# vLAR-group/unMORE

Measured on AMD Instinct MI355X. Metric: images/sec (train fwd+bwd) ObjectnessNet ViT-B/16 384x384, higher is better.
Workload: dtype bf16

## Files before the change

### unmore_amd/csrc/gemm_nt256p.hip

```cpp
#include "umr_common.h"
#include "gemm_epilogue.h"
#include <stdio.h>
#include <stdlib.h>
#include <type_traits>

namespace {

constexpr int BM2 = 256, BN2 = 256, BK2 = 64;
constexpr int ROWB2 = 128;
constexpr int TILE2 = 256 * ROWB2;
constexpr int BUF2 = 2 * TILE2;
constexpr int STG_OFF = 2 * BUF2;
constexpr int STG_BYTES = 32 * 256 * 4;
constexpr int LDS2P = STG_OFF + STG_BYTES;

typedef bf16_t T2;

__device__ __forceinline__ unsigned mul_dgelu_bf16x2(unsigned g, unsigned x) {
    const float lo = __builtin_bit_cast(float, g << 16) * dgelu_sel<bf16_t>(__builtin_bit_cast(float, x << 16));
    const float hi = __builtin_bit_cast(float, g & 0xFFFF0000u) * dgelu_sel<bf16_t>(__builtin_bit_cast(float, x & 0xFFFF0000u));
    typedef __attribute__((ext_vector_type(2))) __bf16 bf16x2;
    bf16x2 r;
    r[0] = (bf16_t)lo; r[1] = (bf16_t)hi;
    return __builtin_bit_cast(unsigned, r);
// ... 313 lines not shown
        QUADRANT_HID(0, fb0, (void)0, (void)0)
        END_SYNC_N(2);
    };
    auto tile_body4_ahead = [&](const char* sbuf) {
#pragma unroll
        for (int ks = 0; ks < 2; ++ks) {
#pragma unroll
            for (int i = 0; i < 2; ++i) fb0[ks][i] = B_FRAG(ks, i);
#pragma unroll
            for (int i = 0; i < 4; ++i) fa[ks][i] = A_FRAG(ks, i);
        }
        READ_WAIT();
        QUADRANT(0, 0, fb0, 1)
        END_SYNC_N(6);
#pragma unroll
        for (int ks = 0; ks < 2; ++ks)
#pragma unroll
            for (int i = 0; i < 2; ++i) fb1[ks][i] = B_FRAG(ks, 2 + i);
        READ_WAIT();
        QUADRANT(0, 2, fb1, 2)
        END_SYNC_N(6);
#pragma unroll
        for (int ks = 0; ks < 2; ++ks)
#pragma unroll
            for (int i = 0; i < 4; ++i) fa[ks][i] = A_FRAG(ks, 4 + i);
        READ_WAIT();
        QUADRANT(4, 2, fb1, 3)
        END_SYNC_N(6);
        stage_prep();
        QUADRANT(4, 0, fb0, 0)
        END_SYNC_N(6);
    };

    if (PRIO_MODE == 1 && w >= 4) __builtin_amdgcn_s_setprio(1);
    stage_setup(0);
    stage_prep();
    STAGE_DMA(0, 0); STAGE_DMA(0, 1); STAGE_DMA(1, 0); STAGE_DMA(1, 1);
    STAGE_DMA(2, 0); STAGE_DMA(2, 1); STAGE_DMA(3, 0); STAGE_DMA(3, 1);
    if (ahead) {
        if (PH2) {
            asm volatile("s_waitcnt vmcnt(2)" ::: "memory");
        } else {
            stage_prep();
            STAGE_DMA(0, 0); STAGE_DMA(0, 1);
            asm volatile("s_waitcnt vmcnt(6)" ::: "memory");
        }
    } else {
        stage_prep();
        STAGE_DMA(0, 0); STAGE_DMA(0, 1); STAGE_DMA(1, 0); STAGE_DMA(1, 1);
        if (PH2) { STAGE_DMA(2, 0); STAGE_DMA(2, 1); }
        asm volatile("s_waitcnt vmcnt(8)" ::: "memory");
    }
    __builtin_amdgcn_s_barrier();

    const int er = lane >> 3, ec = lane & 7;
    const unsigned co_lane = ((unsigned)((w >> 2) * 128 + er) * (unsigned)p.ldc + (unsigned)((w & 3) * 64 + ec * 8)) * 2u;
    const unsigned ax_lane = ((unsigned)((w >> 2) * 128 + er) * (unsigned)p.ldaux + (unsigned)((w & 3) * 64 + ec * 8)) * 2u;
    constexpr int WST_BYTES = 2048;
    constexpr int RW_OFF = 8 * WST_BYTES;
    float* stg = (float*)(smem + STG_OFF);
    auto stage_rows = [&](auto mtag) {
        constexpr int MT = decltype(mtag)::value;
        const int lr = wr * 16 + frow;
#pragma unroll
        for (int ntl = 0; ntl < 4; ++ntl) {
            const int ch = (wc * 16 + ntl * 4 + fq) ^ frow;
            *(f32x4*)(stg + lr * 256 + ch * 4) = acc[MT][ntl];
        }
    };
    int c_par = 0;
    constexpr bool BIAS_INIT = (EPI == 3 || EPI == 4 || EPI == 5 || EPI == 6);
    f32x4 bqn[4];
    auto fetch_bias = [&](int it_) {
        const int v_ = it_ * G + pw;
        const int tn_ = v_ - (v_ / tiles_n) * tiles_n;
#pragma unroll
        for (int ntl = 0; ntl < 4; ++ntl) {
            const int n = tn_ * BN2 + wc * 64 + ntl * 16 + fq * 4;
            bqn[ntl] = f32x4{0.f, 0.f, 0.f, 0.f};
            if ((p.flags & UMR_EPI_BIAS) && it_ < n_my && n < p.N) bqn[ntl] = *(const f32x4*)(p.bias + n);
        }
    };
    if (BIAS_INIT) fetch_bias(0);
#pragma unroll 1
    for (int it = 0; it < n_my; ++it) {
#pragma unroll
        for (int i = 0; i < 8; ++i)
#pragma unroll
            for (int j = 0; j < 4; ++j) acc[i][j] = BIAS_INIT ? bqn[j] : f32x4{0.f, 0.f, 0.f, 0.f};
        if (RED && w < 2) {
            const int v_ = it * G + pw;
            const int n0_ = (v_ - (v_ / tiles_n) * tiles_n) * BN2;
            const __amdgpu_buffer_rsrc_t rsW = __builtin_amdgcn_make_buffer_rsrc(
                (void*)(p.red_w + (int64_t)w * p.N + n0_), 0, (w < p.red_c) ? clamp31((int64_t)(p.N - n0_) * 4) : 0, 0x00020000);
            const int rw_off = (EPI == 3) ? RW_OFF + (it & 1) * 2048 : 0;
            __builtin_amdgcn_raw_ptr_buffer_load_lds(rsW, UMR_LDS_PTR(smem + STG_OFF + rw_off + w * 1024), 16, (unsigned)(lane * 16), 0, 0, 0);
        }
        if (ahead) {
#pragma unroll 1
            for (int t = 0; t < nt; ++t) {
                if (PH2) tile_body2_ahead(smem + c_par * BUF2); else tile_body4_ahead(smem + c_par * BUF2);
                c_par ^= 1;
            }
        } else {
#pragma unroll 1
            for (int t = 0; t < nt; ++t) {
                tile_body(smem + c_par * BUF2);
                c_par ^= 1;
            }
        }
        const int v = it * G + pw;
        const int tm = v / tiles_n, tn = v - tm * tiles_n;
        const int m0 = tm * bm, n0 = tn * BN2;
        const int m_end = (p.M - m0 < bm) ? p.M : m0 + bm;
        if (EPI == 3) {
            fetch_bias(it + 1);
            typedef __attribute__((ext_vector_type(2))) short s16x2;
            typedef __attribute__((ext_vector_type(2))) unsigned u32x2;
            const short relu_lo = (p.act == UMR_ACT_RELU) ? (short)0 : (short)-32768;
            const s16x2 relu16 = {relu_lo, relu_lo};
            auto pack4 = [&](const f32x4& v) -> u32x2 {
                unsigned lo, hi;
                asm("v_cvt_pk_bf16_f32 %0, %1, %2" : "=v"(lo) : "v"(v[0]), "v"(v[1]));
                asm("v_cvt_pk_bf16_f32 %0, %1, %2" : "=v"(hi) : "v"(v[2]), "v"(v[3]));
                s16x2 a = __builtin_bit_cast(s16x2, lo), b = __builtin_bit_cast(s16x2, hi);
                if (AUXM == 0) {
                    a = __builtin_elementwise_max(a, relu16);
                    b = __builtin_elementwise_max(b, relu16);
                }
                return u32x2{__builtin_bit_cast(unsigned, a), __builtin_bit_cast(unsigned, b)};
            };
            bf16x8 rwh[2], rwl[2];
            float* ro_lane = nullptr;
            if (RED) {
#pragma unroll
                for (int pr = 0; pr < 2; ++pr) {
                    f32x4 a = {0.f, 0.f, 0.f, 0.f}, b = {0.f, 0.f, 0.f, 0.f};
                    if (frow < 2) {
                        const char* rwp = smem + STG_OFF + RW_OFF + (it & 1) * 2048 + frow * 1024;
                        a = *(const f32x4*)(rwp + (wc * 64 + (2 * pr) * 16 + fq * 4) * 4);
                        b = *(const f32x4*)(rwp + (wc * 64 + (2 * pr + 1) * 16 + fq * 4) * 4);
                    }
#pragma unroll
                    for (int e = 0; e < 8; ++e) {
                        const float x = e < 4 ? a[e] : b[e - 4];
                        const bf16_t hi = (bf16_t)x;
                        rwh[pr][e] = hi;
                        rwl[pr][e] = (bf16_t)(x - (float)hi);
                    }
                }
                if (fq == 0 && n0 + wc * 64 < p.N)
                    ro_lane = p.red_out + ((int64_t)(tn * 4 + wc) * p.M + (m0 + wr * 128 + frow)) * p.red_c;
            }
            auto row_reduce2 = [&](const bf16x8& a01, const bf16x8& a23, const bf16x8& b01, const bf16x8& b23, int mt_) {
                const f32x4 z = {0.f, 0.f, 0.f, 0.f};
                f32x4 ra = __builtin_amdgcn_mfma_f32_16x16x32_bf16(rwh[0], a01, z, 0, 0, 0);
                f32x4 rb = __builtin_amdgcn_mfma_f32_16x16x32_bf16(rwh[0], b01, z, 0, 0, 0);
                ra = __builtin_amdgcn_mfma_f32_16x16x32_bf16(rwl[0], a01, ra, 0, 0, 0);
                rb = __builtin_amdgcn_mfma_f32_16x16x32_bf16(rwl[0], b01, rb, 0, 0, 0);
                ra = __builtin_amdgcn_mfma_f32_16x16x32_bf16(rwh[1], a23, ra, 0, 0, 0);
                rb = __builtin_amdgcn_mfma_f32_16x16x32_bf16(rwh[1], b23, rb, 0, 0, 0);
                ra = __builtin_amdgcn_mfma_f32_16x16x32_bf16(rwl[1], a23, ra, 0, 0, 0);
                rb = __builtin_amdgcn_mfma_f32_16x16x32_bf16(rwl[1], b23, rb, 0, 0, 0);
                const int m = m0 + wr * 128 + mt_ * 16 + frow;
                if (ro_lane != nullptr) {
                    float* ro = ro_lane + (int64_t)(mt_ * 16) * p.red_c;
// ... 182 lines not shown
            fetch_bias(it + 1);
            const float relu_floor = (p.act == UMR_ACT_RELU) ? 0.f : -INFINITY;
            const bool planes = (p.flags & UMR_EPI_OUT_X3) != 0;
            const bool maskf = (p.flags & UMR_EPI_MASK_RELU) != 0;
            const bool maskp = (p.flags & UMR_EPI_AUX_X3) != 0;
            if (RED) {
                f32x4 rw[2][4];
#pragma unroll
                for (int c = 0; c < 2; ++c)
#pragma unroll
                    for (int ntl = 0; ntl < 4; ++ntl)
                        rw[c][ntl] = *(const f32x4*)(smem + STG_OFF + c * 1024 + (wc * 64 + ntl * 16 + fq * 4) * 4);
#pragma unroll
                for (int mt = 0; mt < 8; ++mt) {
                    float rs0 = 0.f, rs1 = 0.f;
#pragma unroll
                    for (int ntl = 0; ntl < 4; ++ntl) {
                        const f32x4 v = acc[mt][ntl];
#pragma unroll
                        for (int e = 0; e < 4; ++e) {
                            const float t = fmaxf(v[e], relu_floor);
                            rs0 += t * rw[0][ntl][e];
                            rs1 += t * rw[1][ntl][e];
                        }
                    }
                    rs0 += __shfl_xor(rs0, 16, 64); rs0 += __shfl_xor(rs0, 32, 64);
                    rs1 += __shfl_xor(rs1, 16, 64); rs1 += __shfl_xor(rs1, 32, 64);
                    const int m = m0 + wr * 128 + mt * 16 + frow;
                    if (fq == 0 && m < m_end && n0 + wc * 64 < p.N) {
                        float* ro = p.red_out + ((int64_t)(tn * 4 + wc) * p.M + m) * p.red_c;
                        ro[0] = rs0;
                        if (p.red_c == 2) ro[1] = rs1;
                    }
                }
            } else {
#pragma unroll 1
            for (int mt = 0; mt < 8; ++mt) {
                if (mt > 0) __syncthreads();
                switch (mt) {
                    case 0: stage_rows(std::integral_constant<int, 0>{}); break;
                    case 1: stage_rows(std::integral_constant<int, 1>{}); break;
                    case 2: stage_rows(std::integral_constant<int, 2>{}); break;
                    case 3: stage_rows(std::integral_constant<int, 3>{}); break;
                    case 4: stage_rows(std::integral_constant<int, 4>{}); break;
                    case 5: stage_rows(std::integral_constant<int, 5>{}); break;
                    case 6: stage_rows(std::integral_constant<int, 6>{}); break;
                    default: stage_rows(std::integral_constant<int, 7>{}); break;
                }
                __syncthreads();
                constexpr int UNROLL_J = (EPI == 6) ? 1 : 2;
#pragma clang loop unroll_count(UNROLL_J)
                for (int j = 0; j < 2; ++j) {
                    const int lr = (tid >> 5) + j * 16, cg = tid & 31;
                    const int m = m0 + (lr >> 4) * 128 + mt * 16 + (lr & 15), n = n0 + cg * 8;
                    if (m >= m_end || n >= p.N) continue;
                    const int sw = lr & 15;
                    f32x4 v0 = *(const f32x4*)(stg + lr * 256 + (((2 * cg) ^ sw) << 2));
                    f32x4 v1 = *(const f32x4*)(stg + lr * 256 + (((2 * cg + 1) ^ sw) << 2));
                    if constexpr (EPI == 6) {
                        x3_epilogue_store8<false>(p, m, n, v0, v1);
                    } else {
#pragma unroll
                        for (int e = 0; e < 4; ++e) { v0[e] = fmaxf(v0[e], relu_floor); v1[e] = fmaxf(v1[e], relu_floor); }
                        if (maskf) {
                            f32x4 a0, a1;
                            if (maskp) {
                                const bf16x8 h = *(const bf16x8*)((const T2*)p.aux + (int64_t)m * p.ldaux + n);
                                a0 = f32x4{(float)h[0], (float)h[1], (float)h[2], (float)h[3]};
                                a1 = f32x4{(float)h[4], (float)h[5], (float)h[6], (float)h[7]};
                            } else {
                                const float* ap = (const float*)p.aux + (int64_t)m * p.ldaux + n;
                                a0 = *(const f32x4*)ap; a1 = *(const f32x4*)(ap + 4);
                            }
#pragma unroll
                            for (int e = 0; e < 4; ++e) { v0[e] = a0[e] > 0.f ? v0[e] : 0.f; v1[e] = a1[e] > 0.f ? v1[e] : 0.f; }
                        }
                        const int64_t mo = m + (int64_t)sp * p.M;
                        if (planes) x3_planes_store8((T2*)p.C + mo * p.ldc + n, p.N, v0, v1);
                        else { float* cp = (float*)p.C + mo * p.ldc + n; *(f32x4*)cp = v0; *(f32x4*)(cp + 4) = v1; }
                    }
                }
            }
            }
        } else {
            const bool vec_ok = ((p.N & 7) == 0) && ((p.ldc & 7) == 0) && ((p.ldc2 & 7) == 0) && ((p.ldaux & 7) == 0) &&
                                ((p.ldaux2 & 7) == 0);
#pragma unroll 1
            for (int mt = 0; mt < 8; ++mt) {
                if (mt > 0) __syncthreads();
                switch (mt) {
                    case 0: stage_rows(std::integral_constant<int, 0>{}); break;
                    case 1: stage_rows(std::integral_constant<int, 1>{}); break;
                    case 2: stage_rows(std::integral_constant<int, 2>{}); break;
                    case 3: stage_rows(std::integral_constant<int, 3>{}); break;
                    case 4: stage_rows(std::integral_constant<int, 4>{}); break;
                    case 5: stage_rows(std::integral_constant<int, 5>{}); break;
                    case 6: stage_rows(std::integral_constant<int, 6>{}); break;
                    default: stage_rows(std::integral_constant<int, 7>{}); break;
                }
                __syncthreads();
#pragma unroll 1
                for (int j = 0; j < 2; ++j) {
                    const int lr = (tid >> 5) + j * 16, cg = tid & 31;
                    const int m = m0 + (lr >> 4) * 128 + mt * 16 + (lr & 15), n = n0 + cg * 8;
                    if (m >= m_end || n >= p.N) continue;
                    const int sw = lr & 15;
                    const f32x4 v0 = *(const f32x4*)(stg + lr * 256 + (((2 * cg) ^ sw) << 2));
                    const f32x4 v1 = *(const f32x4*)(stg + lr * 256 + (((2 * cg + 1) ^ sw) << 2));
                    if (vec_ok) {
                        epilogue_store8<T2>(p, m, n, v0, v1);
                    } else {
                        epilogue_store<T2>(p, m, n, v0);
                        if (n + 4 < p.N) epilogue_store<T2>(p, m, n + 4, v1);
                    }
                }
            }
        }
        __syncthreads();
    }
    asm volatile("s_waitcnt vmcnt(0)" ::: "memory");
#undef QUADRANT
#undef QUADRANT_S
#undef QUADRANT_HI
#undef QUADRANT_HID
#undef QUADRANT_SD
#undef QUADRANT_D
#undef MFMA
#undef PHASE_SYNC
#undef PHASE_SYNC_N
#undef STAGE_DMA
#undef READ_WAIT
#undef END_SYNC_N
#undef A_FRAG
#undef B_FRAG
}

__global__ __launch_bounds__(256) void x3_splitk_finish_kernel(const umr_gemm_desc p, const float* __restrict__ slabs, int ksplit, int64_t slab_stride) {
    const int n8 = p.N >> 3;
    const int64_t total = (int64_t)p.M * n8;
    for (int64_t idx = (int64_t)blockIdx.x * blockDim.x + threadIdx.x; idx < total; idx += (int64_t)gridDim.x * blockDim.x) {
        const int m = (int)(idx / n8);
        const int n = (int)(idx - (int64_t)m * n8) * 8;
        const float* q = slabs + (int64_t)m * p.N + n;
        f32x4 v0 = *(const f32x4*)q, v1 = *(const f32x4*)(q + 4);
        for (int s_ = 1; s_ < ksplit; ++s_) {
            const float* qs = q + s_ * slab_stride;
            v0 += *(const f32x4*)qs; v1 += *(const f32x4*)(qs + 4);
        }
        x3_epilogue_store8<true>(p, m, n, v0, v1);
    }
}

int num_cus() {
    static const int n = [] {
        int dev = 0;
        hipDeviceProp_t prop;
        return (hipGetDevice(&dev) == hipSuccess && hipGetDeviceProperties(&prop, dev) == hipSuccess && prop.multiProcessorCount > 0)
                   ? prop.multiProcessorCount : 256;
    }();
    return n;
}

}

bool umr_nt256p_fast_epilogue(const umr_gemm_desc* d) {
    const bool vec_ok = ((d->N & 7) == 0) && ((d->ldc & 7) == 0) && ((d->ldaux & 7) == 0);
    const bool mask = (d->flags & UMR_EPI_MASK_RELU) != 0, add = (d->flags & UMR_EPI_ADD_AUX) != 0;
    return vec_ok && d->c2_mode == 0 && d->c_rows_in <= 0 && d->aux_mod <= 0 &&
           !(d->flags & (UMR_EPI_ROWBIAS | UMR_EPI_ADD_AUX2 | UMR_EPI_OUT_F32 | UMR_EPI_MASK_DGELU)) && !(mask && add) &&
           (d->act == UMR_ACT_NONE || (d->act == UMR_ACT_RELU && !mask && !add));
}
bool umr_nt256p_plain_epilogue(const umr_gemm_desc* d) {
    return umr_nt256p_fast_epilogue(d) && (!d->red_w || (d->conv == 0 && !(d->flags & (UMR_EPI_ADD_AUX | UMR_EPI_MASK_RELU))));
}

static bool umr_nt256p_gelu_epilogue(const umr_gemm_desc* d) {
    const bool vec_ok = ((d->N & 7) == 0) && ((d->ldc & 7) == 0) && ((d->ldaux & 7) == 0) && ((d->ldc2 & 7) == 0);
    const bool dg = (d->flags & UMR_EPI_MASK_DGELU) != 0;
    return vec_ok && (d->c2_mode == 0 || (d->c2_mode == 2 && !dg)) && d->c_rows_in <= 0 && d->aux_mod <= 0 && !d->red_w && !d->no_store &&
           !(d->flags & (UMR_EPI_ROWBIAS | UMR_EPI_ADD_AUX2 | UMR_EPI_OUT_F32 | UMR_EPI_MASK_RELU | UMR_EPI_ADD_AUX)) &&
           ((d->act == UMR_ACT_GELU && !dg) || (d->act == UMR_ACT_NONE && dg));
}

static void x3_plan(const umr_gemm_desc* d, int cus, int npairs, int64_t ws_bytes, int* bm_out, int* ks_out) {
    const int tiles_n = (d->N + BN2 - 1) / BN2;
    const int kt = d->conv == 0 ? d->K / BK2 : 9 * (d->Cin / BK2);
    const int bm_env = umr_opt_or(UMR_OPT_NT256_BM, 0);
    const int64_t slab = (int64_t)d->M * d->N * 4;
    int best_ks = 1, best_bm = BM2;
    double best_cost = 1e300;
    for (int bm = BM2; bm >= (d->conv == 0 ? 192 : BM2); bm -= 32) {
        if (d->conv == 0 && (bm_env == 256 || bm_env == 224 || bm_env == 192) && bm != bm_env) continue;
        const int64_t tiles = (int64_t)((d->M + bm - 1) / bm) * tiles_n;
        for (int ks = 1; ks <= 32 && ks * 2 <= kt + 1; ++ks) {
            if (d->red_w && ks > 1) break;
            if (ks > 1 && ((int64_t)ks * slab > ws_bytes)) break;
            const int per = (kt + ks - 1) / ks;
            if ((kt + per - 1) / per != ks) continue;
            const int64_t rounds = (tiles * ks + cus - 1) / cus;
            const double cost = (double)rounds * (per * npairs * (bm / 256.0) + 8.0) + (ks > 1 ? 8.0 + (double)ks * slab / 4.5e6 : 0.0);
            if (cost < best_cost * (ks > best_ks ? 0.90 : 0.98)) { best_cost = cost; best_ks = ks; best_bm = bm; }
        }
    }
    *bm_out = best_bm;
    *ks_out = best_ks;
}

extern "C" int64_t umr_gemm_nt_x3_workspace(const umr_gemm_desc* d) {
    if (d == nullptr || d->dtype != UMR_BF16X3 || d->M <= 0 || d->N <= 0 || d->K <= 0) return 0;
    int bm, ks;
    x3_plan(d, num_cus(), umr_f32_mode_now() == UMR_F32_X3_FAST ? 3 : 6, (int64_t)1 << 40, &bm, &ks);
    return ks > 1 ? (int64_t)ks * d->M * d->N * 4 : 0;
}

int umr_x3_ksplit_of(const umr_gemm_desc* d, int64_t ws_bytes) {
    if (ws_bytes <= 0) return 1;
    int bm, ks;
    x3_plan(d, num_cus(), umr_f32_mode_now() == UMR_F32_X3_FAST ? 3 : 6, ws_bytes, &bm, &ks);
    return ks;
}

int umr_launch_gemm_nt256p_ws(const umr_gemm_desc* d, void* ws, int64_t ws_bytes, hipStream_t s);
int umr_launch_gemm_nt256p(const umr_gemm_desc* d, hipStream_t s) { return umr_launch_gemm_nt256p_ws(d, nullptr, 0, s); }

int umr_launch_gemm_nt256p_ws(const umr_gemm_desc* d, void* ws, int64_t ws_bytes, hipStream_t s) {
    const int tiles_n = (d->N + BN2 - 1) / BN2;
    const int cus = num_cus();
    constexpr int stagger = 1;
    const int bm_env = umr_opt_or(UMR_OPT_NT256_BM, 0);
    int bm = BM2;
    if (d->conv == 0 && d->dtype == UMR_BF16) {
        if (bm_env == 256 || bm_env == 224 || bm_env == 192) bm = bm_env;
        else if ((int64_t)((d->M + BM2 - 1) / BM2) * tiles_n <= 16ll * cus) {
            double best = 1e300;
            for (int c = 256; c >= 192; c -= 32) {
                const int64_t t = (int64_t)((d->M + c - 1) / c) * tiles_n;
                const double cost = (double)((t + cus - 1) / cus) * (0.25 + 0.75 * c / 256.0);
                if (cost < best - 1e-9) { best = cost; bm = c; }
            }
        }
    }
    const int npairs_x3 = umr_f32_mode_now() == UMR_F32_X3_FAST ? 3 : 6;
    int ksplit = 1;
    if (d->dtype == UMR_BF16X3) x3_plan(d, cus, npairs_x3, ws != nullptr ? ws_bytes : 0, &bm, &ksplit);
    if (d->dtype == UMR_BF16X3 && umr_opt(UMR_OPT_X3_TRACE) != UMR_OPT_UNSET)
        fprintf(stderr, "x3 M=%d N=%d K=%d conv=%d Cin=%d ks=%d bm=%d flags=%u act=%d red=%d\n", d->M, d->N, d->K, d->conv, d->Cin, ksplit, bm,
                (unsigned)d->flags, d->act, d->red_w != nullptr);
    const int tiles_m = (d->M + bm - 1) / bm;
    const int64_t total = (int64_t)tiles_m * tiles_n;
    int64_t kf = total / ((int64_t)cus * 32);
    if (kf < 1) kf = 1;
    if (kf > 8) kf = 8;
    const int budget = umr_cu_budget_now();
    const int cub = (budget > 0 && budget < cus) ? budget : cus;
    if (cub < cus) kf = 1;
    int64_t grid64 = cub * kf;
    if (ksplit > 1) grid64 = (cub + ksplit - 1) / ksplit;
    if (total < grid64) grid64 = total;
    const int grid = (int)grid64;
    dim3 g((unsigned)grid, (unsigned)ksplit), b(512);
    const bool fast_ep = umr_nt256p_fast_epilogue(d);
    const int ph_e = umr_opt(UMR_OPT_NT256_PH2);
    const int kt_steps = (d->conv == 0 ? d->K / BK2 : 9 * (d->Cin / BK2)) * (d->dtype == UMR_BF16X3 ? npairs_x3 : 1) / (ksplit > 1 ? ksplit : 1);
    const bool two = ph_e != UMR_OPT_UNSET ? (ph_e != 0) : (kt_steps >= 8);
#define L256P(CV, EP, AX, RD)                                                                                          \
    do {                                                                                                               \
        if (CV == 1 || two) {                                                                                          \
            UMR_SET_MAX_LDS_ONCE((gemm_nt256p_kernel<CV, EP, AX, RD, false, true>), LDS2P);                            \
            hipLaunchKernelGGL((gemm_nt256p_kernel<CV, EP, AX, RD, false, true>), g, b, LDS2P, s, *d, tiles_n, (int)total, stagger, bm); \
        } else {                                                                                                       \
            UMR_SET_MAX_LDS_ONCE((gemm_nt256p_kernel<0, EP, AX, RD, false, false>), LDS2P);                            \
            hipLaunchKernelGGL((gemm_nt256p_kernel<0, EP, AX, RD, false, false>), g, b, LDS2P, s, *d, tiles_n, (int)total, stagger, bm); \
        }                                                                                                              \
    } while (0)
    if ((d->red_w || d->no_store) && !umr_nt256p_plain_epilogue(d))
        return umr_set_error(UMR_ERR_UNSUPPORTED, "gemm_nt: fused row reduction / no_store needs the fast epilogue class (no aux operand with the reduction)");
    const int auxm = (d->flags & UMR_EPI_ADD_AUX) ? 1 : (d->flags & UMR_EPI_MASK_RELU) ? 2 : 0;
#define L256PX(CV, EP)                                                                                                 \
    do {                                                                                                               \
        if (CV == 1 || two) {                                                                                          \
            UMR_SET_MAX_LDS_ONCE((gemm_nt256p_kernel<CV, EP, 0, false, true, true>), LDS2P);                           \
            hipLaunchKernelGGL((gemm_nt256p_kernel<CV, EP, 0, false, true, true>), g, b, LDS2P, s, *d, tiles_n, (int)total, stagger, bm, npairs, 0); \
        } else {                                                                                                       \
            UMR_SET_MAX_LDS_ONCE((gemm_nt256p_kernel<0, EP, 0, false, true, false>), LDS2P);                           \
            hipLaunchKernelGGL((gemm_nt256p_kernel<0, EP, 0, false, true, false>), g, b, LDS2P, s, *d, tiles_n, (int)total, stagger, bm, npairs, 0); \
        }                                                                                                              \
    } while (0)
    if (d->dtype == UMR_BF16X3) {
        const int npairs = npairs_x3;
        if (d->red_w) {
            if (two) {
                UMR_SET_MAX_LDS_ONCE((gemm_nt256p_kernel<0, 5, 0, true, true, true>), LDS2P);
                hipLaunchKernelGGL((gemm_nt256p_kernel<0, 5, 0, true, true, true>), g, b, LDS2P, s, *d, tiles_n, (int)total, stagger, bm, npairs, 0);
            } else {
                UMR_SET_MAX_LDS_ONCE((gemm_nt256p_kernel<0, 5, 0, true, true, false>), LDS2P);
                hipLaunchKernelGGL((gemm_nt256p_kernel<0, 5, 0, true, true, false>), g, b, LDS2P, s, *d, tiles_n, (int)total, stagger, bm, npairs, 0);
            }
        } else if (ksplit > 1) {
            umr_gemm_desc sd = *d;
            sd.C = ws; sd.ldc = d->N; sd.C2 = nullptr; sd.c2_mode = 0; sd.bias = nullptr; sd.aux = nullptr; sd.aux2 = nullptr; sd.rowbias = nullptr;
            sd.flags = UMR_EPI_OUT_F32; sd.act = UMR_ACT_NONE; sd.c_rows_in = 0; sd.aux_mod = 0;
            const umr_gemm_desc* dd = &sd;
            const int kt_all = d->conv == 0 ? d->K / BK2 : 9 * (d->Cin / BK2);
            const int kt_per = (kt_all + ksplit - 1) / ksplit;
#define L256PXS(CV)                                                                                                    \
    do {                                                                                                               \
        if (CV == 1 || two) {                                                                                          \
            UMR_SET_MAX_LDS_ONCE((gemm_nt256p_kernel<CV, 5, 0, false, true, true>), LDS2P);                            \
            hipLaunchKernelGGL((gemm_nt256p_kernel<CV, 5, 0, false, true, true>), g, b, LDS2P, s, *dd, tiles_n, (int)total, stagger, bm, npairs, kt_per); \
        } else {                                                                                                       \
            UMR_SET_MAX_LDS_ONCE((gemm_nt256p_kernel<0, 5, 0, false, true, false>), LDS2P);                            \
            hipLaunchKernelGGL((gemm_nt256p_kernel<0, 5, 0, false, true, false>), g, b, LDS2P, s, *dd, tiles_n, (int)total, stagger, bm, npairs, kt_per); \
        }                                                                                                              \
    } while (0)
            if (d->conv == 0) L256PXS(0); else L256PXS(1);
#undef L256PXS
            UMR_LAUNCH_CHECK();
            const int64_t tasks = (int64_t)d->M * (d->N >> 3);
            int64_t fg = (tasks + 255) / 256;
            if (fg > 8192) fg = 8192;
            hipLaunchKernelGGL(x3_splitk_finish_kernel, dim3((unsigned)fg), dim3(256), 0, s, *d, (const float*)ws, ksplit, (int64_t)d->M * d->N);
        } else {
            const bool lean = !(d->flags & ~(UMR_EPI_BIAS | UMR_EPI_OUT_F32 | UMR_EPI_OUT_X3 | UMR_EPI_MASK_RELU | UMR_EPI_AUX_X3)) && d->c2_mode == 0 &&
                              d->c_rows_in <= 0 && d->aux_mod <= 0 && d->act != UMR_ACT_GELU;
            if (d->conv == 0) { if (lean) L256PX(0, 5); else L256PX(0, 6); }
            else { if (lean) L256PX(1, 5); else L256PX(1, 6); }
        }
        UMR_LAUNCH_CHECK();
        return UMR_OK;
    }
#undef L256PX
    if (d->conv == 0) {
        if (fast_ep) {
            if (d->red_w) L256P(0, 3, 0, true);
            else if (auxm == 0) L256P(0, 3, 0, false);
            else if (auxm == 1) L256P(0, 3, 1, false);
            else L256P(0, 3, 2, false);
        } else if (umr_nt256p_gelu_epilogue(d)) { if (d->flags & UMR_EPI_MASK_DGELU) L256P(0, 4, 2, false); else L256P(0, 4, 0, false); }
        else L256P(0, 1, 0, false);
    } else {
        if (fast_ep) {
            if (auxm == 0) L256P(1, 3, 0, false);
            else if (auxm == 1) L256P(1, 3, 1, false);
            else L256P(1, 3, 2, false);
        } else L256P(1, 1, 0, false);
    }
#undef L256P
    UMR_LAUNCH_CHECK();
    return UMR_OK;
}
```

### unmore_amd/csrc/gemm_tn256.hip

```cpp
#include "umr_common.h"
#include <type_traits>
#include <stdlib.h>

namespace {

constexpr int TSUB = 64 * 256;
constexpr int TBUF = 4 * TSUB;
constexpr int TLDS = 2 * TBUF;

__device__ __forceinline__ int tn_swz2(int r) { return ((r & 3) << 2) | ((r >> 2) & 3); }

template <int CONV, bool PH2, int WF, bool X3 = false>
__global__ __launch_bounds__(512, 2) void gemm_tn256_kernel(const umr_gemm_tn_desc p, int tiles_k, int ntiles, int rows_per_split,
                                                            float* slab, float* bslab, int mapmode, int npairs_arg = 1) {
    extern __shared__ __attribute__((aligned(16))) char smem[];
    constexpr int SZ = 2;
    const int npairs = X3 ? npairs_arg : 1;
    const int xpix = X3 ? 3 * p.Cin : p.Cin;
    constexpr unsigned OOB = 0x80000000u;
    const int tid = threadIdx.x, lane = tid & 63;
    const int w = __builtin_amdgcn_readfirstlane(tid >> 6);
    int bid = blockIdx.x;
    {
        const int nwg = gridDim.x, xcd = bid & 7, q_ = nwg >> 3, r_ = nwg & 7;
// ... 233 lines not shown
    auto stage_body = [&]() {
        if (PH2) { stage_body2(); return; }
#pragma unroll
        for (int t = 0; t < 2; ++t) { fx0[0][t] = RF(1, 0, x_ad[t]); fx0[1][t] = RF(1, 1, x_ad[t]); }
#pragma unroll
        for (int t = 0; t < 4; ++t) { fy[0][t] = RF(0, 0, y_ad[t]); fy[1][t] = RF(0, 1, y_ad[t]); }
        PHASE_SYNC();
        BIAS_ACC(0)
        QUADRANT(0, 0, fx0, 2)
#pragma unroll
        for (int t = 0; t < 2; ++t) { fx1[0][t] = RF(2, 0, x_ad[t]); fx1[1][t] = RF(2, 1, x_ad[t]); }
        PHASE_SYNC();
        QUADRANT(0, 2, fx1, 3)
        stage_prep();
#pragma unroll
        for (int t = 0; t < 4; ++t) { fy[0][t] = RF(3, 0, y_ad[t]); fy[1][t] = RF(3, 1, y_ad[t]); }
        PHASE_SYNC();
        BIAS_ACC(4)
        QUADRANT(4, 2, fx1, 0)
        PHASE_SYNC();
        QUADRANT(4, 0, fx0, 1)
    };

    if (PRIO_MODE == 1 && w >= 4) __builtin_amdgcn_s_setprio(1);
    stage_prep();
    STAGE_DMA(0, 0); STAGE_DMA(0, 1); STAGE_DMA(1, 0); STAGE_DMA(1, 1);
    STAGE_DMA(2, 0); STAGE_DMA(2, 1); STAGE_DMA(3, 0); STAGE_DMA(3, 1);
    stage_prep();
    STAGE_DMA(0, 0); STAGE_DMA(0, 1); STAGE_DMA(1, 0); STAGE_DMA(1, 1);
    if (PH2) { STAGE_DMA(2, 0); STAGE_DMA(2, 1); }
    asm volatile("s_waitcnt vmcnt(8)" ::: "memory");
    __builtin_amdgcn_s_barrier();

    int bias_next = tk;
    int c_pp = 0, c_m = 0;
    const int nsteps = nst * npairs;
#pragma unroll 1
    for (int t = 0; t < nsteps; ++t) {
        par_off = lds0 + (unsigned)((t & 1) * TBUF);
        const bool sum_pair = !X3 || ((((npairs == 6 ? 0x124 : 0x004) >> (2 * c_pp)) & 3) == 0);
        bias_turn = (c_m == bias_next) && sum_pair;
        stage_body();
        if (++c_pp == npairs) { c_pp = 0; if (c_m == bias_next) bias_next += tiles_k; ++c_m; }
    }
#undef BIAS_ACC
#undef QUADRANT
#undef QUADRANT_D
#undef PHASE_SYNC_N
#undef MFMA
#undef PHASE_SYNC
#undef STAGE_DMA
#undef RF
    asm volatile("s_waitcnt vmcnt(0)" ::: "memory");

    float* out = slab + (int64_t)split * p.N * p.K;
#pragma unroll
    for (int nt = 0; nt < 8; ++nt) {
        const int n = (mapmode & 2) ? n0 + (nt >> 2) * 128 + wn * 64 + (nt & 3) * 16 + li : n0 + wn * 128 + nt * 16 + li;
        if (n >= p.N) continue;
#pragma unroll
        for (int kt = 0; kt < 4; ++kt) {
            const int k = (mapmode & 1) ? k0 + (kt >> 1) * 128 + wk * 32 + (kt & 1) * 16 + g * 4 : k0 + wk * 64 + kt * 16 + g * 4;
            if (k >= p.K) continue;
            float* o = out + (int64_t)n * p.K + k;
            if (k + 3 < p.K && (p.K & 3) == 0) *(f32x4*)o = acc[nt][kt];
            else { for (int e = 0; e < 4; ++e) if (k + e < p.K) o[e] = acc[nt][kt][e]; }
        }
        if (do_bias && wk == 0) {
            float s_ = bsum[nt];
            s_ += __shfl_xor(s_, 16, 64);
            s_ += __shfl_xor(s_, 32, 64);
            if (g == 0) bslab[((int64_t)split * tiles_k + tk) * p.N + n] = s_;
        }
    }
}

}

bool umr_tn256_eligible(const umr_gemm_tn_desc* d, bool force) {
    if (d->dtype != UMR_BF16 && d->dtype != UMR_BF16X3) return false;
    if (d->dy_rows_in > 0 || d->x_rows_in > 0) return false;
    if (d->conv == 2) return false;
    if (d->dtype == UMR_BF16X3) return true;
    if (d->conv == 1 && d->Wo < 64) return false;
    if (force) return true;
    if (d->N < 192 || d->K < 192) return false;
    const int64_t tiles = (int64_t)((d->N + 255) / 256) * ((d->K + 255) / 256);
    return (int64_t)d->M >= 256 * 64 * 16 / (tiles < 1 ? 1 : tiles) && d->M >= 64 * 64;
}

void umr_tn256_plan(const umr_gemm_tn_desc* d, int* splits, int* rows_per_split) {
    const int64_t tiles = (int64_t)((d->N + 255) / 256) * ((d->K + 255) / 256);
    const int x3 = d->dtype == UMR_BF16X3 ? 6 : 1;
    int64_t rounds = (int64_t)d->M * tiles * x3 / (256ll * 4096);
    if (rounds < 1) rounds = 1;
    if (rounds > 4) rounds = 4;
    int64_t want = rounds * 256 / tiles;
    if (want < 1) want = 1;
    const int64_t min_stages = x3 == 6 ? 2 : 16;
    const int64_t max_by_rows = ((int64_t)d->M + 64 * min_stages - 1) / (64 * min_stages);
    if (want > max_by_rows) want = max_by_rows;
    int64_t rps = ((int64_t)d->M + want - 1) / want;
    rps = (rps + 63) / 64 * 64;
    {
        const int64_t cpix = (int64_t)d->Cin * (d->dtype == UMR_BF16X3 ? 3 : 1);
        const int64_t rowb = 2 * (int64_t)(d->conv ? (cpix > d->lddy ? cpix : d->lddy) : (d->ldx > d->lddy ? d->ldx : d->lddy));
        const int64_t halo = d->conv ? (2 * (int64_t)d->W + 4) * cpix * 2 : 0;
        int64_t cap = ((1ll << 31) - halo - 65536) / rowb / 64 * 64;
        if (cap < 64) cap = 64;
        if (rps > cap) rps = cap;
    }
    *rows_per_split = (int)rps;
    *splits = (int)(((int64_t)d->M + rps - 1) / rps);
}

int umr_launch_gemm_tn256(const umr_gemm_tn_desc* d, int splits, int rows_per_split, float* slab, float* bslab, hipStream_t s) {
    const int tiles_n = (d->N + 255) / 256, tiles_k = (d->K + 255) / 256;
    dim3 g((unsigned)(tiles_n * tiles_k * splits)), b(512);
    constexpr int mapmode = 3;
#define LT(CV, WFV)                                                                                                    \
    do {                                                                                                               \
        UMR_SET_MAX_LDS_ONCE((gemm_tn256_kernel<CV, true, WFV>), TLDS);                                                \
        hipLaunchKernelGGL((gemm_tn256_kernel<CV, true, WFV>), g, b, TLDS, s, *d, tiles_k, tiles_n * tiles_k, rows_per_split, slab, bslab, mapmode, 1); \
    } while (0)
#define LTX(CV, WFV)                                                                                                   \
    do {                                                                                                               \
        UMR_SET_MAX_LDS_ONCE((gemm_tn256_kernel<CV, true, WFV, true>), TLDS);                                          \
        hipLaunchKernelGGL((gemm_tn256_kernel<CV, true, WFV, true>), g, b, TLDS, s, *d, tiles_k, tiles_n * tiles_k, rows_per_split, slab, bslab, mapmode, npairs); \
    } while (0)
    if (d->dtype == UMR_BF16X3) {
        const int npairs = umr_f32_mode_now() == UMR_F32_X3_FAST ? 3 : 6;
        if (d->conv == 0) LTX(0, 0);
        else if (d->Wo % 64 == 0) LTX(1, 1);
        else if (d->Wo >= 64) LTX(1, 0);
        else LTX(1, 2);
    } else if (d->conv == 0) LT(0, 0);
    else if (d->Wo % 64 == 0) LT(1, 1);
    else LT(1, 0);
#undef LTX
#undef LT
    UMR_LAUNCH_CHECK();
    return UMR_OK;
}
```

### unmore_amd/csrc/umr_api.hip

```cpp
#include "umr_common.h"
#include <string.h>

static thread_local char g_err[256] = "";

int umr_set_error(int code, const char* msg) {
    strncpy(g_err, msg ? msg : "", sizeof(g_err) - 1);
    g_err[sizeof(g_err) - 1] = 0;
    return code;
}

extern "C" int umr_version(void) { return 100; }
extern "C" const char* umr_last_error_string(void) { return g_err; }

#include <atomic>
#include <stdlib.h>
static std::atomic<int> g_f32_mode{-1};
int umr_f32_mode_now() {
    int m = g_f32_mode.load(std::memory_order_relaxed);
    if (m < 0) {
        const char* e = getenv("UMR_F32_X3");
        m = (e && atoi(e) == 0) ? UMR_F32_EXACT : UMR_F32_X3;
        g_f32_mode.store(m, std::memory_order_relaxed);
    }
    return m;
}
extern "C" int umr_set_f32_mode(int mode) {
    if (mode != UMR_F32_EXACT && mode != UMR_F32_X3 && mode != UMR_F32_X3_FAST) return umr_set_error(UMR_ERR_INVALID, "umr_set_f32_mode: unknown mode");
    g_f32_mode.store(mode, std::memory_order_relaxed);
    return UMR_OK;
}
extern "C" int umr_get_f32_mode(void) { return umr_f32_mode_now(); }

static std::atomic<int> g_cu_budget{-1};
int umr_cu_budget_now() {
    int b = g_cu_budget.load(std::memory_order_relaxed);
    if (b < 0) {
        const char* e = getenv("UMR_CU_BUDGET");
        b = e ? atoi(e) : 0;
        if (b < 0) b = 0;
        g_cu_budget.store(b, std::memory_order_relaxed);
    }
    return b;
}
extern "C" int umr_set_cu_budget(int cus) {
    if (cus < 0) return umr_set_error(UMR_ERR_INVALID, "umr_set_cu_budget: negative budget");
    g_cu_budget.store(cus, std::memory_order_relaxed);
    return UMR_OK;
}
extern "C" int umr_get_cu_budget(void) { return umr_cu_budget_now(); }

static const char* const g_opt_names[UMR_OPT_COUNT] = {
    "UMR_GEMM_TILE", "UMR_NT_SPLITK", "UMR_SPLITK_FENCE", "UMR_NT_ORDER", "UMR_NT256_PERSIST", "UMR_NT256_BM",
    "UMR_X3_TRACE", "UMR_NT256_PH2", "UMR_ATTN_BWD_FUSED", "UMR_BILINEAR_GY", "UMR_HEAD_OUT_BWD_GENERIC"};
static std::atomic<int> g_opt[UMR_OPT_COUNT];
static int opt_parse(const char* v) {
    if (!v) return UMR_OPT_UNSET;
    if ((v[0] >= '0' && v[0] <= '9') || v[0] == '-' || v[0] == '+') return atoi(v);
    return (int)(unsigned char)v[0];
}
static const bool g_opt_loaded = [] {
    for (int i = 0; i < UMR_OPT_COUNT; ++i) g_opt[i].store(opt_parse(getenv(g_opt_names[i])), std::memory_order_relaxed);
    return true;
}();
int umr_opt(int id) { return g_opt[id].load(std::memory_order_relaxed); }
extern "C" int umr_set_debug_option(const char* name, const char* value) {
    if (!name) return umr_set_error(UMR_ERR_INVALID, "umr_set_debug_option: null name");
    for (int i = 0; i < UMR_OPT_COUNT; ++i)
        if (strcmp(name, g_opt_names[i]) == 0) {
            g_opt[i].store(opt_parse(value), std::memory_order_relaxed);
            return UMR_OK;
        }
    return umr_set_error(UMR_ERR_INVALID, "umr_set_debug_option: unknown option");
}
extern "C" int umr_get_debug_option(const char* name, int* value, int* is_set) {
    if (!name) return umr_set_error(UMR_ERR_INVALID, "umr_get_debug_option: null name");
    for (int i = 0; i < UMR_OPT_COUNT; ++i)
        if (strcmp(name, g_opt_names[i]) == 0) {
            const int v = g_opt[i].load(std::memory_order_relaxed);
            if (is_set) *is_set = v != UMR_OPT_UNSET;
            if (value) *value = v == UMR_OPT_UNSET ? 0 : v;
            return UMR_OK;
        }
    return umr_set_error(UMR_ERR_INVALID, "umr_get_debug_option: unknown option");
}
```

### unmore_amd/csrc/umr_common.h

```cpp
#pragma once
#include <hip/hip_runtime.h>
#include <stdint.h>
#include "../../include/umr.h"

typedef __bf16 bf16_t;
typedef __attribute__((ext_vector_type(8))) __bf16 bf16x8;
typedef __attribute__((ext_vector_type(4))) __bf16 bf16x4;
typedef __attribute__((ext_vector_type(2))) __bf16 bf16x2;
typedef __attribute__((ext_vector_type(4))) float f32x4;
typedef __attribute__((ext_vector_type(2))) float f32x2;
typedef __attribute__((ext_vector_type(16))) float f32x16;
typedef __attribute__((ext_vector_type(2))) unsigned u32x2;
typedef __attribute__((ext_vector_type(4))) unsigned u32x4;

#define UMR_GLOBAL_PTR(p) ((const __attribute__((address_space(1))) void*)(p))
#define UMR_LDS_PTR(p) ((__attribute__((address_space(3))) void*)(p))

__device__ __forceinline__ void glds16(const void* gsrc, void* lds_wave_base) {
    __builtin_amdgcn_global_load_lds(UMR_GLOBAL_PTR(gsrc), UMR_LDS_PTR(lds_wave_base), 16, 0, 0);
}

template <typename T> __device__ __forceinline__ float to_f32(T v);
template <> __device__ __forceinline__ float to_f32<float>(float v) { return v; }
template <> __device__ __forceinline__ float to_f32<bf16_t>(bf16_t v) { return (float)v; }
template <typename T> __device__ __forceinline__ T from_f32(float v);
template <> __device__ __forceinline__ float from_f32<float>(float v) { return v; }
template <> __device__ __forceinline__ bf16_t from_f32<bf16_t>(float v) { return (bf16_t)v; }

template <typename T> struct Vec4;
template <> struct Vec4<float> {
    static __device__ __forceinline__ f32x4 load(const float* p) { return *(const f32x4*)p; }
    static __device__ __forceinline__ void store(float* p, f32x4 v) { *(f32x4*)p = v; }
};
template <> struct Vec4<bf16_t> {
    static __device__ __forceinline__ f32x4 load(const bf16_t* p) {
        bf16x4 t = *(const bf16x4*)p;
        f32x4 r = {(float)t[0], (float)t[1], (float)t[2], (float)t[3]};
        return r;
    }
    static __device__ __forceinline__ void store(bf16_t* p, f32x4 v) {
        bf16x4 t = {(bf16_t)v[0], (bf16_t)v[1], (bf16_t)v[2], (bf16_t)v[3]};
        *(bf16x4*)p = t;
    }
};

__device__ __forceinline__ float gelu_erf(float x) { return 0.5f * x * (1.0f + erff(x * 0.70710678118654752440f)); }
__device__ __forceinline__ float dgelu_erf(float x) {
    const float cdf = 0.5f * (1.0f + erff(x * 0.70710678118654752440f));
    const float pdf = 0.39894228040143267794f * __expf(-0.5f * x * x);
    return cdf + x * pdf;
}

__device__ __forceinline__ void erf_exp_fast(float x, float& erf_z, float& e) {
    const float z = fabsf(x) * 0.70710678118654752440f;
    const float t = __builtin_amdgcn_rcpf(1.0f + 0.3275911f * z);
    e = __builtin_amdgcn_exp2f(-0.72134752044448170368f * x * x);
    const float poly = t * (0.254829592f + t * (-0.284496736f + t * (1.421413741f + t * (-1.453152027f + t * 1.061405429f))));
    const float r = 1.0f - poly * e;
    erf_z = x < 0.f ? -r : r;
}
template <typename T> __device__ __forceinline__ float gelu_sel(float x) {
    if constexpr (sizeof(T) == 2) {
        float ez, e;
        erf_exp_fast(x, ez, e);
        return 0.5f * x * (1.0f + ez);
    } else {
        return gelu_erf(x);
    }
}
template <typename T> __device__ __forceinline__ float dgelu_sel(float x) {
    if constexpr (sizeof(T) == 2) {
        float ez, e;
        erf_exp_fast(x, ez, e);
        return 0.5f * (1.0f + ez) + x * 0.39894228040143267794f * e;
    } else {
        return dgelu_erf(x);
    }
}

__device__ __forceinline__ float wave_sum(float v) {
#pragma unroll
    for (int o = 32; o > 0; o >>= 1) v += __shfl_xor(v, o, 64);
    return v;
}
__device__ __forceinline__ float wave_max(float v) {
#pragma unroll
    for (int o = 32; o > 0; o >>= 1) v = fmaxf(v, __shfl_xor(v, o, 64));
    return v;
}

static __device__ uint4 umr_zero_page[16];

#include <atomic>
#define UMR_SET_MAX_LDS_ONCE(fn, bytes)                                                                             \
    do {                                                                                                            \
        static std::atomic<bool> done_{false};                                                                      \
        if (!done_.load(std::memory_order_acquire)) {                                                               \
            (void)hipFuncSetAttribute((const void*)(fn), hipFuncAttributeMaxDynamicSharedMemorySize, (bytes));      \
            done_.store(true, std::memory_order_release);                                                           \
        }                                                                                                           \
    } while (0)

#include <limits.h>
enum {
    UMR_OPT_GEMM_TILE = 0, UMR_OPT_NT_SPLITK, UMR_OPT_SPLITK_FENCE, UMR_OPT_NT_ORDER, UMR_OPT_NT256_PERSIST, UMR_OPT_NT256_BM,
    UMR_OPT_X3_TRACE, UMR_OPT_NT256_PH2, UMR_OPT_ATTN_BWD_FUSED, UMR_OPT_BILINEAR_GY, UMR_OPT_HEAD_OUT_BWD_GENERIC, UMR_OPT_COUNT
};
#define UMR_OPT_UNSET INT_MIN
int umr_opt(int id);
static inline int umr_opt_or(int id, int dflt) { const int v = umr_opt(id); return v == UMR_OPT_UNSET ? dflt : v; }

int umr_set_error(int code, const char* msg);
int umr_f32_mode_now();
int umr_cu_budget_now();
#define UMR_CHECK_ARG(cond, msg) do { if (!(cond)) return umr_set_error(UMR_ERR_INVALID, msg); } while (0)
#define UMR_LAUNCH_CHECK() do { hipError_t e_ = hipGetLastError(); if (e_ != hipSuccess) return umr_set_error(UMR_ERR_HIP - (int)e_, hipGetErrorString(e_)); } while (0)
```

Baseline: 354.1.

## Add specialized decoder epilogue to NT256 GEMM and optional narrow-conv TN256 path

Adds an EPI==7 epilogue variant to the persistent 256x256 NT GEMM for decoder patterns (bias plus aux add or ReLU mask, a second aux add, optional dual ReLU store). It stages accumulators per wave through LDS, prefetches aux tiles with buffer loads two row blocks ahead, and prefetches bias for the next tile, replacing the generic row-staged epilogue with its block-wide syncs. It also adds an opt-in env switch that lets narrow conv (Wo<64) use the TN256 kernel with a new template variant. The change adds more template instantiations and code size, and relies on the vector-alignment checks for correctness.

```diff
diff --git a/unmore_amd/csrc/gemm_nt256p.hip b/unmore_amd/csrc/gemm_nt256p.hip
--- a/unmore_amd/csrc/gemm_nt256p.hip
+++ b/unmore_amd/csrc/gemm_nt256p.hip
@@ -419,6 +419,14 @@
         }
     };
     if (BIAS_INIT) fetch_bias(0);
+    f32x4 bco[2];
+    auto fetch_bias_co = [&](int it_) {
+        const int v_ = it_ * G + pw;
+        const int n = (v_ - (v_ / tiles_n) * tiles_n) * BN2 + wc * 64 + ec * 8;
+        bco[0] = bco[1] = f32x4{0.f, 0.f, 0.f, 0.f};
+        if ((p.flags & UMR_EPI_BIAS) && it_ < n_my && n < p.N) { bco[0] = *(const f32x4*)(p.bias + n); bco[1] = *(const f32x4*)(p.bias + n + 4); }
+    };
+    if (EPI == 7) fetch_bias_co(0);
 #pragma unroll 1
     for (int it = 0; it < n_my; ++it) {
 #pragma unroll
@@ -767,6 +775,95 @@
                 }
             }
             }
+        } else if (EPI == 7) {
+            constexpr int XM = AUXM & 3;
+            constexpr bool X2 = (AUXM & 4) != 0, TWO = (AUXM & 8) != 0;
+            const bool has_bias = (p.flags & UMR_EPI_BIAS) != 0;
+            const f32x4 bc0 = bco[0], bc1 = bco[1];
+            fetch_bias_co(it + 1);
+            const bool col_live = n0 + wc * 64 + ec * 8 < p.N;
+            const int rows_live = m_end - m0;
+            auto tile_rsrc = [&](const void* base, int64_t ld) {
+                return __builtin_amdgcn_make_buffer_rsrc((void*)((T2*)base + (int64_t)m0 * ld + n0), 0, clamp31((int64_t)rows_live * ld * 2), 0x00020000);
+            };
+            auto lane_off = [&](int64_t ld) -> unsigned {
+                return col_live ? ((unsigned)(wr * 128 + er) * (unsigned)ld + (unsigned)(wc * 64 + ec * 8)) * 2u : OOB;
+            };
+            const __amdgpu_buffer_rsrc_t rsC = tile_rsrc(p.C, p.ldc);
+            const __amdgpu_buffer_rsrc_t rsC2 = TWO ? tile_rsrc(p.C2, p.ldc2) : rsC;
+            const __amdgpu_buffer_rsrc_t rsX = XM != 0 ? tile_rsrc(p.aux, p.ldaux) : rsC;
+            const __amdgpu_buffer_rsrc_t rsX2 = X2 ? tile_rsrc(p.aux2, p.ldaux2) : rsC;
+            const unsigned co_vo = lane_off(p.ldc), c2_vo = TWO ? lane_off(p.ldc2) : OOB;
+            const unsigned ax_vo = XM != 0 ? lane_off(p.ldaux) : OOB, ax2_vo = X2 ? lane_off(p.ldaux2) : OOB;
+            u32x4 axc[4][2], ax2c[4][2];
+            auto load_auxc = [&](auto btag) {
+                constexpr int MB = decltype(btag)::value;
+                if (MB < 8) {
+#pragma unroll
+                    for (int k = 0; k < 2; ++k) {
+                        if (XM != 0) axc[MB & 3][k] = __builtin_amdgcn_raw_buffer_load_b128(rsX, ax_vo + (unsigned)((MB * 16 + k * 8) * p.ldaux * 2), 0, 0);
+                        if (X2) ax2c[MB & 3][k] = __builtin_amdgcn_raw_buffer_load_b128(rsX2, ax2_vo + (unsigned)((MB * 16 + k * 8) * p.ldaux2 * 2), 0, 0);
+                    }
+                }
+            };
+            load_auxc(std::integral_constant<int, 0>{});
+            load_auxc(std::integral_constant<int, 1>{});
+            char* wst = smem + STG_OFF + w * (2 * WST_BYTES);
+            char* wst_w = wst + frow * 256;
+            const char* wst_r[2] = {wst + er * 256, wst + (er + 8) * 256};
+            auto widen = [](const u32x4& a, f32x4& lo, f32x4& hi) {
+                const bf16x8 t = __builtin_bit_cast(bf16x8, a);
+                lo = f32x4{(float)t[0], (float)t[1], (float)t[2], (float)t[3]};
+                hi = f32x4{(float)t[4], (float)t[5], (float)t[6], (float)t[7]};
+            };
+            auto narrow = [](const f32x4& lo, const f32x4& hi) -> u32x4 {
+                bf16x8 t;
+                t[0] = (bf16_t)lo[0]; t[1] = (bf16_t)lo[1]; t[2] = (bf16_t)lo[2]; t[3] = (bf16_t)lo[3];
+                t[4] = (bf16_t)hi[0]; t[5] = (bf16_t)hi[1]; t[6] = (bf16_t)hi[2]; t[7] = (bf16_t)hi[3];
+                return __builtin_bit_cast(u32x4, t);
+            };
+            auto block7 = [&](auto btag) {
+                constexpr int MB = decltype(btag)::value;
+                load_auxc(std::integral_constant<int, MB + 2>{});
+#pragma unroll
+                for (int ntl = 0; ntl < 4; ++ntl) *(f32x4*)(wst_w + (((ntl * 4 + fq) ^ frow) << 4)) = acc[MB][ntl];
+                asm volatile("" ::: "memory");
+                f32x4 v[2][2];
+#pragma unroll
+                for (int k = 0; k < 2; ++k)
+#pragma unroll
+                    for (int h = 0; h < 2; ++h) v[k][h] = *(const f32x4*)(wst_r[k] + (((2 * ec + h) ^ (er + 8 * k)) << 4));
+                asm volatile("" ::: "memory");
+#pragma unroll
+                for (int k = 0; k < 2; ++k) {
+                    f32x4 v0 = v[k][0], v1 = v[k][1];
+                    if (has_bias) { v0 += bc0; v1 += bc1; }
+                    if (XM != 0) {
+                        f32x4 a0, a1;
+                        widen(axc[MB & 3][k], a0, a1);
+                        if (XM == 1) { v0 += a0; v1 += a1; }
+                        else {
+#pragma unroll
+                            for (int j = 0; j < 4; ++j) { v0[j] = a0[j] > 0.f ? v0[j] : 0.f; v1[j] = a1[j] > 0.f ? v1[j] : 0.f; }
+                        }
+                    }
+                    if (X2) {
+                        f32x4 a0, a1;
+                        widen(ax2c[MB & 3][k], a0, a1);
+                        v0 += a0; v1 += a1;
+                    }
+                    __builtin_amdgcn_raw_buffer_store_b128(narrow(v0, v1), rsC, co_vo + (unsigned)((MB * 16 + k * 8) * p.ldc * 2), 0, 0);
+                    if (TWO) {
+#pragma unroll
+                        for (int j = 0; j < 4; ++j) { v0[j] = fmaxf(v0[j], 0.f); v1[j] = fmaxf(v1[j], 0.f); }
+                        __builtin_amdgcn_raw_buffer_store_b128(narrow(v0, v1), rsC2, c2_vo + (unsigned)((MB * 16 + k * 8) * p.ldc2 * 2), 0, 0);
+                    }
+                }
+            };
+            block7(std::integral_constant<int, 0>{}); block7(std::integral_constant<int, 1>{});
+            block7(std::integral_constant<int, 2>{}); block7(std::integral_constant<int, 3>{});
+            block7(std::integral_constant<int, 4>{}); block7(std::integral_constant<int, 5>{});
+            block7(std::integral_constant<int, 6>{}); block7(std::integral_constant<int, 7>{});
         } else {
             const bool vec_ok = ((p.N & 7) == 0) && ((p.ldc & 7) == 0) && ((p.ldc2 & 7) == 0) && ((p.ldaux & 7) == 0) &&
                                 ((p.ldaux2 & 7) == 0);
@@ -857,6 +954,18 @@
 }
 bool umr_nt256p_plain_epilogue(const umr_gemm_desc* d) {
     return umr_nt256p_fast_epilogue(d) && (!d->red_w || (d->conv == 0 && !(d->flags & (UMR_EPI_ADD_AUX | UMR_EPI_MASK_RELU))));
+}
+
+static int umr_nt256p_decoder_epilogue(const umr_gemm_desc* d) {
+    if (umr_opt_or(UMR_OPT_NT256_EPI_GENERIC, 0) != 0) return -1;
+    const bool vec_ok = ((d->N & 7) == 0) && ((d->ldc & 7) == 0) && ((d->ldc2 & 7) == 0) && ((d->ldaux & 7) == 0) && ((d->ldaux2 & 7) == 0);
+    if (!vec_ok || d->c_rows_in > 0 || d->aux_mod > 0 || d->red_w || d->no_store || d->act != UMR_ACT_NONE || d->c2_mode > 1 ||
+        (d->flags & (UMR_EPI_ROWBIAS | UMR_EPI_OUT_F32 | UMR_EPI_MASK_DGELU)))
+        return -1;
+    const bool mask = (d->flags & UMR_EPI_MASK_RELU) != 0, add = (d->flags & UMR_EPI_ADD_AUX) != 0, add2 = (d->flags & UMR_EPI_ADD_AUX2) != 0;
+    if (mask && add) return -1;
+    const int code = (add ? 1 : mask ? 2 : 0) | (add2 ? 4 : 0) | (d->c2_mode == 1 ? 8 : 0);
+    return (code == 8 || code == 5 || code == 13 || code == 6) ? code : -1;
 }
 
 static bool umr_nt256p_gelu_epilogue(const umr_gemm_desc* d) {
@@ -1015,21 +1124,32 @@
         return UMR_OK;
     }
 #undef L256PX
+    const int dec = fast_ep ? -1 : umr_nt256p_decoder_epilogue(d);
+#define L256P_DEC(CV)                                                                                                  \
+    do {                                                                                                               \
+        if (dec == 8) L256P(CV, 7, 8, false);                                                                          \
+        else if (dec == 5) L256P(CV, 7, 5, false);                                                                     \
+        else if (dec == 13) L256P(CV, 7, 13, false);                                                                   \
+        else L256P(CV, 7, 6, false);                                                                                   \
+    } while (0)
     if (d->conv == 0) {
         if (fast_ep) {
             if (d->red_w) L256P(0, 3, 0, true);
             else if (auxm == 0) L256P(0, 3, 0, false);
             else if (auxm == 1) L256P(0, 3, 1, false);
             else L256P(0, 3, 2, false);
-        } else if (umr_nt256p_gelu_epilogue(d)) { if (d->flags & UMR_EPI_MASK_DGELU) L256P(0, 4, 2, false); else L256P(0, 4, 0, false); }
+        } else if (dec >= 0) L256P_DEC(0);
+        else if (umr_nt256p_gelu_epilogue(d)) { if (d->flags & UMR_EPI_MASK_DGELU) L256P(0, 4, 2, false); else L256P(0, 4, 0, false); }
         else L256P(0, 1, 0, false);
     } else {
         if (fast_ep) {
             if (auxm == 0) L256P(1, 3, 0, false);
             else if (auxm == 1) L256P(1, 3, 1, false);
             else L256P(1, 3, 2, false);
-        } else L256P(1, 1, 0, false);
+        } else if (dec >= 0) L256P_DEC(1);
+        else L256P(1, 1, 0, false);
     }
+#undef L256P_DEC
 #undef L256P
     UMR_LAUNCH_CHECK();
     return UMR_OK;
diff --git a/unmore_amd/csrc/gemm_tn256.hip b/unmore_amd/csrc/gemm_tn256.hip
--- a/unmore_amd/csrc/gemm_tn256.hip
+++ b/unmore_amd/csrc/gemm_tn256.hip
@@ -339,7 +339,7 @@
     if (d->dy_rows_in > 0 || d->x_rows_in > 0) return false;
     if (d->conv == 2) return false;
     if (d->dtype == UMR_BF16X3) return true;
-    if (d->conv == 1 && d->Wo < 64) return false;
+    if (d->conv == 1 && d->Wo < 64 && umr_opt_or(UMR_OPT_TN_NARROW_256, 0) == 0) return false;
     if (force) return true;
     if (d->N < 192 || d->K < 192) return false;
     const int64_t tiles = (int64_t)((d->N + 255) / 256) * ((d->K + 255) / 256);
@@ -393,7 +393,8 @@
         else LTX(1, 2);
     } else if (d->conv == 0) LT(0, 0);
     else if (d->Wo % 64 == 0) LT(1, 1);
-    else LT(1, 0);
+    else if (d->Wo >= 64) LT(1, 0);
+    else LT(1, 2);
 #undef LTX
 #undef LT
     UMR_LAUNCH_CHECK();
diff --git a/unmore_amd/csrc/umr_api.hip b/unmore_amd/csrc/umr_api.hip
--- a/unmore_amd/csrc/umr_api.hip
+++ b/unmore_amd/csrc/umr_api.hip
@@ -51,7 +51,8 @@
 
 static const char* const g_opt_names[UMR_OPT_COUNT] = {
     "UMR_GEMM_TILE", "UMR_NT_SPLITK", "UMR_SPLITK_FENCE", "UMR_NT_ORDER", "UMR_NT256_PERSIST", "UMR_NT256_BM",
-    "UMR_X3_TRACE", "UMR_NT256_PH2", "UMR_ATTN_BWD_FUSED", "UMR_BILINEAR_GY", "UMR_HEAD_OUT_BWD_GENERIC"};
+    "UMR_X3_TRACE", "UMR_NT256_PH2", "UMR_ATTN_BWD_FUSED", "UMR_BILINEAR_GY", "UMR_HEAD_OUT_BWD_GENERIC",
+    "UMR_TN_NARROW_256", "UMR_NT256_EPI_GENERIC"};
 static std::atomic<int> g_opt[UMR_OPT_COUNT];
 static int opt_parse(const char* v) {
     if (!v) return UMR_OPT_UNSET;
diff --git a/unmore_amd/csrc/umr_common.h b/unmore_amd/csrc/umr_common.h
--- a/unmore_amd/csrc/umr_common.h
+++ b/unmore_amd/csrc/umr_common.h
@@ -104,7 +104,8 @@
 #include <limits.h>
 enum {
     UMR_OPT_GEMM_TILE = 0, UMR_OPT_NT_SPLITK, UMR_OPT_SPLITK_FENCE, UMR_OPT_NT_ORDER, UMR_OPT_NT256_PERSIST, UMR_OPT_NT256_BM,
-    UMR_OPT_X3_TRACE, UMR_OPT_NT256_PH2, UMR_OPT_ATTN_BWD_FUSED, UMR_OPT_BILINEAR_GY, UMR_OPT_HEAD_OUT_BWD_GENERIC, UMR_OPT_COUNT
+    UMR_OPT_X3_TRACE, UMR_OPT_NT256_PH2, UMR_OPT_ATTN_BWD_FUSED, UMR_OPT_BILINEAR_GY, UMR_OPT_HEAD_OUT_BWD_GENERIC,
+    UMR_OPT_TN_NARROW_256, UMR_OPT_NT256_EPI_GENERIC, UMR_OPT_COUNT
 };
 #define UMR_OPT_UNSET INT_MIN
 int umr_opt(int id);
```

Result: no change. 356.8, median of 6 (+0.7%).
